# tobiasleibner/dune-hdd

Hardware: AMD Instinct MI355X
Metric: assembled DoFs/sec (global stiffness), SPE10 SWIPDG p=1 (higher is better)
Workload: dtype f64

## Files before the change

dune-hdd_amd/csrc/host/grid.cpp:

```cpp
#include <algorithm>
#include <cmath>
#include <cstring>
#include <fstream>
#include <memory>
#include <numeric>
#include <string>
#include <vector>

#include "hdd.h"
#include "hdd_internal.hh"

namespace hdd {

static const int kSimplexFV[3][2] = {{0, 1}, {0, 2}, {1, 2}};
static const int kCubeFV[4][2] = {{0, 2}, {1, 3}, {0, 1}, {2, 3}};

static inline const int (*face_table(int et))[2] { return et == HDD_SIMPLEX ? kSimplexFV : kCubeFV; }
static inline int nvpe_of(int et) { return et == HDD_SIMPLEX ? 3 : 4; }

static inline double linspace_node(double a, double b, int64_t n, int64_t i)
{
  if (i == n) return b;
  const double step = (b - a) / double(n);
  return double(i) * step + a;
// ... 467 lines not shown
      const double lo = vertex_coords[3 * v[0] + c], hi = vertex_coords[3 * v[1 << c] + c];
      if (!(hi > lo)) return set_error(HDD_ERR_UNSUPPORTED, std::string(fn) + ": element " + std::to_string(e) +
                                                             " is not an axis-aligned box in Dune vertex order");
      for (int k = 0; k < 8; ++k) {
        const double want = ((k >> c) & 1) ? hi : lo, x = vertex_coords[3 * v[k] + c];
        if (std::fabs(x - want) > 1e-12 * std::max(std::fabs(hi - lo), std::fabs(want)))
          return set_error(HDD_ERR_UNSUPPORTED, std::string(fn) + ": element " + std::to_string(e) +
                                                    " is not an axis-aligned box in Dune vertex order");
      }
    }
  }
  auto G = std::make_unique<ExplicitGrid>();
  G->elem_type = HDD_HEX;
  G->dim = 3;
  G->nvpe = 8;
  G->nf = 6;
  G->nb = int(nb);
  return finish_explicit(std::move(G), n_vertices, vertex_coords, n_elements, elem_vert, subdomain, n_subdomains,
                         boundary, out, fn);
}

extern "C" void hdd_grid_destroy(hdd_grid* g) { delete g; }

extern "C" int hdd_grid_get_info(const hdd_grid* g, hdd_grid_info* out)
{
  if (!g || !out) return set_error(HDD_ERR_INVALID, "hdd_grid_get_info: null argument");
  const Grid& G = *g->impl;
  out->elem_type = G.elem_type;
  out->nb = G.nb;
  out->nfaces = G.nf;
  out->nvpe = G.nvpe;
  out->n_elements = G.ne;
  out->n_vertices = G.nv;
  out->n_subdomains = G.n_sub;
  out->dim = G.dim;
  return HDD_OK;
}

extern "C" int hdd_grid_subdomain_range(const hdd_grid* g, int32_t s_begin, int32_t s_end, int64_t* first,
                                        int64_t* last)
{
  if (!g || !first || !last) return set_error(HDD_ERR_INVALID, "hdd_grid_subdomain_range: null argument");
  const Grid& G = *g->impl;
  if (s_begin < 0 || s_end > G.n_sub || s_begin >= s_end)
    return set_error(HDD_ERR_RANGE, "hdd_grid_subdomain_range: 0 <= s_begin < s_end <= num_subdomains violated");
  *first = G.sub_first[s_begin];
// ... 403 lines not shown
```

dune-hdd_amd/csrc/host/hdd_internal.hh:

```
#pragma once
#include <string>

#include "hdd.h"

namespace hdd {
std::string& last_error_slot();
const char*& last_tile_kernel_slot();
int set_error(int code, const std::string& msg);
int ctx_device(const hdd_ctx* ctx);
}

int hdd_fix_rb(int32_t elem_type);
int hdd_assemble_elements_buf(hdd_ctx* ctx, const hdd_mesh* m, const hdd_scalar_fn* kappa, int32_t n_comp,
                              const hdd_tensor_fn* tensor, const hdd_swipdg_params* p, const hdd_csr* pattern,
                              double* const* d_bufs, const int32_t* d_elems, int64_t n_elems, void* stream);
int hdd_scatter_fix(hdd_ctx* ctx, const hdd_csr* pattern, int32_t rb, double* const* d_bufs, int32_t n_comp,
                    const int32_t* d_elems, int64_t n_elems, double* const* d_vals, void* stream);
int hdd_assemble_elements_soa(hdd_ctx* ctx, const hdd_mesh* m, const hdd_scalar_fn* kappa, int32_t n_comp,
                              const hdd_tensor_fn* tensor, const hdd_swipdg_params* p, const hdd_csr* pattern,
                              double* const* d_bufs, int64_t ld, const int32_t* d_elems, int64_t n_elems, void* stream);
int hdd_scatter_fix_q1_soa(hdd_ctx* ctx, const hdd_mesh* m, const hdd_csr* pattern, double* const* d_bufs, int64_t ld,
                           int32_t n_comp, const int32_t* d_elems, int64_t n_elems, double* const* d_vals, void* stream);
int hdd_assemble_reserve(hdd_ctx* ctx, const hdd_mesh* m, const hdd_scalar_fn* kappa, int32_t n_comp,
                         const hdd_tensor_fn* tensor, const hdd_swipdg_params* p, const hdd_csr* pattern,
                         double* const* d_vals, void* stream, int32_t reserve_wg);
int hdd_assemble_elements_inplace(hdd_ctx* ctx, const hdd_mesh* m, const hdd_scalar_fn* kappa, int32_t n_comp,
                                  const hdd_tensor_fn* tensor, const hdd_swipdg_params* p, const hdd_csr* pattern,
                                  double* const* d_vals, const int32_t* d_elems, int64_t n_elems, void* stream);
int hdd_assemble_skip_ghost(hdd_ctx* ctx, const hdd_mesh* m, const hdd_scalar_fn* kappa, int32_t n_comp,
                            const hdd_tensor_fn* tensor, const hdd_swipdg_params* p, const hdd_csr* pattern,
                            double* const* d_vals, void* stream, int32_t reserve_wg = 0);
```

dune-hdd_amd/csrc/kernels/abi_assemble.hip:

```cpp
#include <hip/hip_runtime.h>

#include <algorithm>
#include <cstdint>
#include <string>
#include <vector>

#include "abi_common.hh"
#include "quadrature.hh"

using hdd::set_error;
using namespace hdd::abi;

namespace {
const char* const WHO = "hdd_swipdg_assemble";

struct AssembleMode {
  const int32_t* list = nullptr;
  int64_t n_list = 0;
  int32_t list_kind = hdd::dev::LIST_TILES;
  bool skip_ghost = false;
  int32_t reserve_wg = 0;
  int64_t fix_ld = 0;
};
}

static int assemble_hex(hdd_ctx* ctx, const hdd_mesh* m, const hdd_scalar_fn* kappa, int32_t n_comp,
                        const hdd_tensor_fn* tensor, const hdd_swipdg_params* p, const hdd_csr* pattern,
                        double* const* d_vals, void* stream)
{
  using namespace hdd::dev;
  int deg = 1;
  if (int rc = check_degree(WHO, m, &deg)) return rc;
  if (int rc = check_pattern_rows(WHO, pattern, mesh_nb(HDD_HEX, deg), m)) return rc;
  if (int rc = check_tensor_kind(WHO, tensor)) return rc;
  if (int rc = check_tensor(WHO, tensor)) return rc;
  hipError_t e = hipSetDevice(ctx->device);
  if (e != hipSuccess) return hip_fail(e, "hdd_swipdg_assemble: hipSetDevice");
  for (int c = 0; c < n_comp; ++c) {
    const hdd_scalar_fn& k = kappa[c];
    if (k.kind != HDD_FN_CONST && k.kind != HDD_FN_PER_ELEM && k.kind != HDD_FN_SINUSOID)
      return fail(HDD_ERR_UNSUPPORTED, WHO, "unknown diffusion factor kind");
    if (int rc = check_fn_per_elem(WHO, &k)) return rc;
    if (!d_vals[c]) return fail(HDD_ERR_INVALID, WHO, "null value array");
    const int ko = fn_order(k);
    const int vol_order = p->vol_order >= 0 ? p->vol_order : ko + 2 * (deg - 1);
// ... 72 lines not shown
      return set_error(HDD_ERR_UNSUPPORTED, "hdd_swipdg_assemble_tiles: no tile / element lists for HDD_HEX");
    return assemble_hex(ctx, m, kappa, n_comp, tensor, p, pattern, d_vals, stream);
  }
  int deg = 1;
  if (int rc = check_degree(WHO, m, &deg)) return rc;
  if (int rc = check_pattern_rows(WHO, pattern, mesh_nb(m->elem_type, deg), m)) return rc;
  if (int rc = check_tensor_kind(WHO, tensor)) return rc;
  if (int rc = check_tensor(WHO, tensor)) return rc;
  AssembleArgs a = mesh_args(ctx, m, pattern);
  set_coefficients(a, tensor, p);
  a.n_comp = n_comp;
  a.tile_list = mode.list;
  a.n_tile_list = mode.n_list;
  a.list_elements = mode.list_kind;
  a.skip_ghost = mode.skip_ghost ? 1 : 0;
  a.reserve_wg = mode.list_kind != LIST_TILES ? 0 : mode.reserve_wg;
  a.fix_ld = mode.fix_ld;
  a.fix_rb = hdd_fix_rb(m->elem_type);
  if (int rc = check_vertex_arrays(WHO, m)) return rc;
  if (use_vertex_geometry(ctx, m, false, true)) {
    a.ev = m->elem_vertices;
    a.vxy = m->vertex_coords;
  }
  const int ko = fn_order(kappa[0]);
  for (int c = 0; c < n_comp; ++c) {
    const hdd_scalar_fn& k = kappa[c];
    if (k.kind != HDD_FN_CONST && k.kind != HDD_FN_PER_ELEM && k.kind != HDD_FN_SINUSOID && k.kind != HDD_FN_FLATTOP)
      return fail(HDD_ERR_UNSUPPORTED, WHO, "unknown diffusion factor kind");
    if (int rc = check_fn_per_elem(WHO, &k)) return rc;
    if (fn_order(k) != ko) return fail(HDD_ERR_UNSUPPORTED, WHO, "components of different integration order");
    if (!d_vals[c]) return fail(HDD_ERR_INVALID, WHO, "null value array");
    if (int rc = check_flattop(WHO, &k, m->elem_type, HDD_ERR_INVALID, HDD_ERR_UNSUPPORTED)) return rc;
    a.kappa[c] = KappaArg{k.kind, k.order, k.c, k.b, k.kx, k.ky, k.per_elem, k.table, k.n_table, 0};
    a.vals[c] = d_vals[c];
  }
  const int vol_order = p->vol_order >= 0 ? p->vol_order : ko;
  const int face_order = p->face_order >= 0 ? p->face_order : ko + 2;
  const int nqv = volume_points(m->elem_type, vol_order);
  const int nqf = face_points(face_order);
  bool supported = false;
  hipError_t e = hipSetDevice(ctx->device);
  if (e != hipSuccess) return hip_fail(e, "hdd_swipdg_assemble: hipSetDevice");
  e = launch_assemble(a, nqv, nqf, static_cast<hipStream_t>(stream), &supported);
  if (!supported)
    return set_error(HDD_ERR_UNSUPPORTED, "hdd_swipdg_assemble: no kernel for volume order " + std::to_string(vol_order) +
                                              " / face order " + std::to_string(face_order));
// ... 86 lines not shown
int hdd_assemble_reserve(hdd_ctx* ctx, const hdd_mesh* m, const hdd_scalar_fn* kappa, int32_t n_comp,
                         const hdd_tensor_fn* tensor, const hdd_swipdg_params* p, const hdd_csr* pattern,
                         double* const* d_vals, void* stream, int32_t reserve_wg)
{
  AssembleMode mode;
  mode.reserve_wg = reserve_wg;
  return assemble_impl(ctx, m, kappa, n_comp, tensor, p, pattern, d_vals, mode, stream);
}

int hdd_scatter_fix_q1_soa(hdd_ctx* ctx, const hdd_mesh* m, const hdd_csr* pattern, double* const* d_bufs, int64_t ld,
                           int32_t n_comp, const int32_t* d_elems, int64_t n_elems, double* const* d_vals, void* stream)
{
  if (n_elems == 0) return HDD_OK;
  hdd::dev::AssembleArgs a = mesh_args(ctx, m, pattern);
  a.tile_list = d_elems;
  a.n_tile_list = n_elems;
  for (int32_t c = 0; c < n_comp; ++c) {
    const hipError_t e = hdd::dev::launch_q1_scatter_soa(a, d_bufs[c], ld, d_vals[c], static_cast<hipStream_t>(stream));
    if (e != hipSuccess) return hip_fail(e, "hdd_scatter_fix_q1_soa");
  }
  return HDD_OK;
}

int hdd_assemble_skip_ghost(hdd_ctx* ctx, const hdd_mesh* m, const hdd_scalar_fn* kappa, int32_t n_comp,
                            const hdd_tensor_fn* tensor, const hdd_swipdg_params* p, const hdd_csr* pattern,
                            double* const* d_vals, void* stream, int32_t reserve_wg)
{
  AssembleMode mode;
  mode.skip_ghost = true;
  mode.reserve_wg = reserve_wg;
  return assemble_impl(ctx, m, kappa, n_comp, tensor, p, pattern, d_vals, mode, stream);
}

int hdd_scatter_fix(hdd_ctx* ctx, const hdd_csr* pattern, int32_t rb, double* const* d_bufs, int32_t n_comp,
                    const int32_t* d_elems, int64_t n_elems, double* const* d_vals, void* stream)
{
  if (n_elems == 0) return HDD_OK;
  const unsigned grid = unsigned(std::min<int64_t>(n_elems, int64_t(ctx->n_cu) * 8));
  for (int32_t c = 0; c < n_comp; ++c) {
    hipLaunchKernelGGL(fix_scatter_kernel, dim3(grid), dim3(64), 0, static_cast<hipStream_t>(stream), d_bufs[c], rb,
                       d_elems, n_elems, pattern->elem_ptr, d_vals[c]);
    const hipError_t e = hipGetLastError();
    if (e != hipSuccess) return hip_fail(e, "hdd_scatter_fix");
  }
  return HDD_OK;
}
// ... 1 lines not shown
```

dune-hdd_amd/csrc/kernels/ctx.hh:

```
#pragma once
#include <hip/hip_runtime.h>

#include <cstddef>
#include <cstdint>
#include <string>

#include "hdd.h"
#include "../host/hdd_internal.hh"

#pragma GCC visibility push(hidden)

struct DeviceScratch {
  enum Slack { EXACT, QUARTER };
  enum SyncBeforeFree { NO_SYNC, SYNC_STREAM, SYNC_DEVICE };
  void* p = nullptr;
  size_t bytes = 0;
  const bool pinned_host;

  explicit DeviceScratch(bool pinned_host_ = false) : pinned_host(pinned_host_) {}
  DeviceScratch(const DeviceScratch&) = delete;
  DeviceScratch& operator=(const DeviceScratch&) = delete;
  ~DeviceScratch() { release(); }

  hipError_t reserve(size_t need, Slack slack, SyncBeforeFree sync, hipStream_t s = nullptr)
// ... 32 lines not shown
  int wgcu = 0;
  int q3g_reps = 0;
  double* q3g_tab = nullptr;
  DeviceScratch scan_ws;
  DeviceScratch ops_d;
  DeviceScratch ops_h{true};
  hipEvent_t ops_evt = nullptr;
  int64_t* nnz_h = nullptr;
  int64_t* nnz_hd = nullptr;
  DeviceScratch rhs_ws;
  hipStream_t rhs_stream = nullptr;
  hipEvent_t rhs_evt = nullptr;
  bool rhs_used = false;

  ~hdd_ctx()
  {
    if (q3g_tab) (void)hipFree(q3g_tab);
    if (nnz_h) (void)hipHostFree(nnz_h);
    if (rhs_evt) (void)hipEventDestroy(rhs_evt);
    if (ops_evt) (void)hipEventDestroy(ops_evt);
  }
};

inline bool vx_offsets_fit(int64_t n_local) { return n_local >= 0 && n_local * 48 < (int64_t(1) << 32); }

inline int hip_fail(hipError_t e, const char* where)
{
  return hdd::set_error(HDD_ERR_HIP, std::string(where) + ": " + hipGetErrorString(e));
}

#pragma GCC visibility pop
```

dune-hdd_amd/csrc/kernels/shard.hip:

```cpp
#include <hip/hip_runtime.h>
#include <rccl/rccl.h>

#include <dlfcn.h>

#include <algorithm>
#include <chrono>
#include <condition_variable>
#include <cstdint>
#include <cstring>
#include <map>
#include <mutex>
#include <string>
#include <thread>
#include <vector>

#include "hdd.h"
#include "../host/hdd_internal.hh"

using hdd::set_error;

namespace {

int hip_fail(hipError_t e, const char* where)
{
// ... 591 lines not shown
  if (c->direct && c->direct == static_cast<hipStream_t>(stream)) {
    c->direct = nullptr;
    return HDD_OK;
  }
  hipError_t e = hipSetDevice(c->device);
  if (e == hipSuccess) e = hipStreamWaitEvent(static_cast<hipStream_t>(stream), c->done, 0);
  return e == hipSuccess ? HDD_OK : hip_fail(e, "hdd_comm_wait");
}

struct hdd_shard {
  int device = 0;
  hdd_local* local = nullptr;
  hdd_grid_info gi{};
  hdd_local_info li{};
  int32_t rank = 0, nranks = 1, s_begin = 0, s_end = 0, degree = 1;
  int64_t nnz = 0;
  std::vector<int64_t> gid;
  double* d_coords = nullptr;
  int32_t* d_nbrs = nullptr;
  uint32_t* d_finfo = nullptr;
  int64_t* d_gid = nullptr;
  int32_t* d_ev = nullptr;
  double* d_vxy = nullptr;
  std::vector<int32_t> peers;
  std::vector<int64_t> send_prefix, recv_prefix, recv_col0;
  int32_t* d_send_idx = nullptr;
  double* d_sbuf = nullptr;
  double* d_rbuf = nullptr;
  int32_t max_rows = 0;
  int32_t* d_tiles_in = nullptr;
  int32_t* d_tiles_bd = nullptr;
  int32_t* d_fix = nullptr;
  int64_t n_tiles = 0, n_in = 0, n_bd = 0, n_fix = 0;
  int64_t halo_faces = 0;
  std::vector<int32_t> send_idx, tiles_in, tiles_bd;
  bool host_only = false;
  hipStream_t aux = nullptr;
  hipEvent_t ev_in = nullptr, ev_out = nullptr;
  double* d_fixbuf = nullptr;
  size_t fixbuf_doubles = 0;
  uint32_t stages = 0;
  hipEvent_t ev_pack = nullptr, ev_xdone = nullptr;
  std::vector<int32_t> stage_peers;
  hipEvent_t ev_mark = nullptr;
  bool marked = false;
};
// ... 70 lines not shown
  std::vector<uint32_t> finfo(static_cast<size_t>(nl));
  sh->gid.resize(size_t(nl));
  rc = hdd_local_fill(sh->local, coords.data(), nbrs.data(), finfo.data(), sh->gid.data(), nullptr);
  if (rc) return fail(rc);
  rc = hdd_dg_pattern_count(gi.nfaces, gi.nb, nl, ob, oe, nbrs.data(), &sh->nnz);
  if (rc) return fail(rc);
  std::vector<int32_t> ev;
  std::vector<double> vxy;
  if (gi.dim == 2) {
    int64_t nvl = 0;
    rc = hdd_local_vertices(sh->local, &nvl, nullptr, nullptr);
    if (rc) return fail(rc);
    ev.resize(size_t(gi.nvpe) * nl);
    vxy.resize(size_t(2) * nvl);
    rc = hdd_local_vertices(sh->local, &nvl, ev.data(), vxy.data());
    if (rc) return fail(rc);
  }

  int32_t np = 0;
  rc = hdd_local_halo_plan(sh->local, own.data(), rank, &np, nullptr, nullptr, nullptr, nullptr);
  if (rc) return fail(rc);
  if (np > SH_MAX_PEERS) return fail(set_error(HDD_ERR_UNSUPPORTED, "hdd_shard_create: more than 64 halo peers"));
  sh->peers.resize(size_t(np));
  std::vector<int64_t> sc(static_cast<size_t>(np)), ro(static_cast<size_t>(np)), rcnt(static_cast<size_t>(np));
  rc = hdd_local_halo_plan(sh->local, own.data(), rank, &np, sh->peers.data(), sc.data(), ro.data(), rcnt.data());
  if (rc) return fail(rc);
  sh->send_prefix.assign(size_t(np) + 1, 0);
  sh->recv_prefix.assign(size_t(np) + 1, 0);
  sh->recv_col0 = ro;
  for (int32_t k = 0; k < np; ++k) {
    sh->send_prefix[k + 1] = sh->send_prefix[k] + sc[k];
    sh->recv_prefix[k + 1] = sh->recv_prefix[k] + rcnt[k];
  }
  std::vector<int32_t> send_idx(size_t(sh->send_prefix[np]));
  for (int32_t k = 0; k < np; ++k) {
    if (!sc[k]) continue;
    rc = hdd_local_send_list(sh->local, own.data(), rank, k, send_idx.data() + sh->send_prefix[k]);
    if (rc) return fail(rc);
  }

  const int64_t n_own = oe - ob;
  sh->n_tiles = (n_own + 63) / 64;
  std::vector<int32_t> tin, tbd, fix;
  for (int64_t t = 0; t < sh->n_tiles; ++t) {
    bool ghost = false;
    for (int64_t e = ob + 64 * t; e < std::min(oe, ob + 64 * t + 64); ++e) {
// ... 162 lines not shown
  }
  const hipStream_t s = static_cast<hipStream_t>(stream);

  HaloArgs h{};
  h.ld = sh->li.n_local;
  h.n_peers = int32_t(sh->peers.size());
  auto add = [&](double* p, int rows) {
    h.arr[h.n_arrays] = p;
    h.row_first[h.n_arrays + 1] = h.row_first[h.n_arrays] + rows;
    ++h.n_arrays;
  };
  if (flags & HDD_SHARD_HALO_GEOMETRY) add(sh->d_coords, sh->gi.dim * sh->gi.nvpe);
  if (tensor->kind == HDD_TENSOR_ISO_PER_ELEM || tensor->kind == HDD_TENSOR_SYM_PER_ELEM) {
    if (!tensor->per_elem) return set_error(HDD_ERR_INVALID, "hdd_block_assemble_sharded: tensor per_elem missing");
    add(const_cast<double*>(tensor->per_elem),
        tensor->kind == HDD_TENSOR_ISO_PER_ELEM ? 1 : (sh->gi.dim == 3 ? 6 : 3));
  }
  for (int32_t c = 0; c < n_comp; ++c)
    if (kappa[c].kind == HDD_FN_PER_ELEM) {
      if (!kappa[c].per_elem) return set_error(HDD_ERR_INVALID, "hdd_block_assemble_sharded: kappa per_elem missing");
      add(const_cast<double*>(kappa[c].per_elem), 1);
    }
  const bool exchange = h.n_peers > 0 && !(flags & HDD_SHARD_NO_HALO) && h.n_arrays > 0;
  if (!exchange) return hdd_swipdg_assemble(ctx, &m, kappa, n_comp, tensor, params, pattern, d_vals, stream);
  const bool transfer = !(flags & HDD_SHARD_NO_TRANSFER);
  if (!comm && transfer)
    return set_error(HDD_ERR_INVALID, "hdd_block_assemble_sharded: the shard has halo peers but comm is NULL");
  const int32_t R = h.row_first[h.n_arrays];
  if (R > sh->max_rows) return set_error(HDD_ERR_INVALID, "hdd_block_assemble_sharded: too many halo rows");

  hipError_t e = hipSetDevice(sh->device);
  if (e != hipSuccess) return hip_fail(e, "hdd_block_assemble_sharded: hipSetDevice");
  sh->stages = 0;
  sh->marked = false;
  const bool default_schedule = !(flags & (HDD_SHARD_FIX_INLINE | HDD_SHARD_FIX_SCATTER | HDD_SHARD_FIX_INPLACE));
  const bool split = (flags & HDD_SHARD_SPLIT_TILES) != 0 ||
                     (default_schedule && sh->gi.elem_type == HDD_SIMPLEX && sh->peers.size() >= 2 && sh->n_in > 0);
  const bool q1_serial = sh->gi.elem_type == HDD_CUBE && default_schedule && !(flags & HDD_SHARD_SPLIT_TILES);
  bool overlap = !(flags & HDD_SHARD_NO_OVERLAP) && sh->gi.elem_type != HDD_HEX && !q1_serial &&
                 (split ? sh->n_in > 0 : true);
  hipStream_t ps = s;
#ifdef HDD_ABLATION
  const bool last = (flags & HDD_SHARD_LAUNCH_LAST) != 0;
#else
  const bool last = false;
#endif
  const bool side = overlap && !split;
// ... 257 lines not shown
```

dune-hdd_amd/csrc/kernels/swipdg_kernels.hh:

```
#pragma once
#include <hip/hip_runtime.h>

#include <cstdint>

#include "hdd.h"

namespace hdd {
namespace dev {

struct KappaArg {
  int32_t kind, order;
  double c, b, kx, ky;
  const double* per_elem;
  const double* table;
  int32_t n_table, pad;
};
__host__ __device__ constexpr bool smooth_kind(int k) { return k == HDD_FN_SINUSOID || k == HDD_FN_FLATTOP; }

enum : int32_t {
  LIST_TILES = 0,
  LIST_ELEMENTS = 1,
  LIST_SIDE_BUFFER = 2,
  LIST_IN_PLACE = 3,
  LIST_SIDE_SOA = 4
};

struct AssembleArgs {
  int32_t elem_type, n_comp;
  int64_t n_local, own_begin, own_end;
  const double* coords;
  const int32_t* nbrs;
  const uint32_t* finfo;
  const int64_t* elem_ptr;
  int32_t tkind, n_cu;
  double tc0, tc1, tc2;
  const double* tper;
  double sigma_inner, sigma_boundary, beta;
  int32_t debug_flags, wgcu;
  uint32_t variant;
  int32_t pad_v;
  const int32_t* tile_list;
  int64_t n_tile_list;
  int32_t list_elements;
  int32_t fix_rb;
  int64_t fix_ld;
  int32_t skip_ghost;
  int32_t reserve_wg;
  const int32_t* ev;
  const double* vxy;
  KappaArg kappa[HDD_MAX_COMP];
  double* vals[HDD_MAX_COMP];
};
inline AssembleArgs component_args(const AssembleArgs& a, int c)
{
  AssembleArgs ac = a;
  ac.n_comp = 1;
  ac.kappa[0] = a.kappa[c];
  ac.vals[0] = a.vals[c];
  return ac;
}
template <bool ALL_IN_ONE, class F>
hipError_t per_component(const AssembleArgs& a, F&& launch)
{
  for (int c = 0; c < (ALL_IN_ONE ? 1 : a.n_comp); ++c) {
    launch(ALL_IN_ONE ? a : component_args(a, c));
    const hipError_t e = hipGetLastError();
    if (e != hipSuccess) return e;
  }
  return hipSuccess;
}

struct HexTables {
// ... 108 lines not shown
```

dune-hdd_amd/csrc/kernels/swipdg_launch.hh:

```
#pragma once
#include <algorithm>
#include <string>
#include <type_traits>

#include "hdd_internal.hh"
#include "swipdg_persistent.hh"

namespace hdd {
namespace dev {

template <class P>
static std::string kernel_name(const char* flags)
{
  const std::string f = __PRETTY_FUNCTION__;
  const size_t a = f.find("P = "), b = f.rfind(']');
  std::string p = a == std::string::npos ? "?" : f.substr(a + 4, b - a - 4);
  if (p.rfind("hdd::dev::", 0) == 0) p = p.substr(10);
  return "swipdg_persistent_kernel<" + p + ", " + flags + ">";
}

template <class P>
static hipError_t launch_persistent(const AssembleArgs& a, hipStream_t s)
{
  const int64_t n_own = a.own_end - a.own_begin;
  if (n_own <= 0) return hipSuccess;
  const int64_t tiles = a.tile_list ? a.n_tile_list : (n_own + 63) / 64;
  if (tiles <= 0) return hipSuccess;
  const size_t lds = (P::PAD ? size_t(image_blocks<P>()) * P::RB : size_t(64) * P::RB + 2 + P::RB) * sizeof(double) *
                     (P::TWO ? 2 : 1);
  if (P::TWO && a.n_comp != 2) return hipErrorInvalidValue;
  const int cus = a.n_cu;
  int wgcu = a.wgcu > 0 ? a.wgcu : P::WGCU;
  size_t lds_launch = lds;
#ifdef HDD_ABLATION
  if (a.wgcu >= 16) {
    lds_launch = std::max(lds, size_t((160 * 1024) / (a.wgcu >> 4)) & ~size_t(15));
    wgcu = (a.wgcu & 15) ? (a.wgcu & 15) : P::WGCU;
  }
#endif
  wgcu = std::max(1, std::min<int>(wgcu, int((160 * 1024) / lds_launch)));
  int64_t slots = int64_t(cus) * wgcu;
  const bool reserve = a.reserve_wg > 0 && !HDD_ABL(a, 4194304);
  if (reserve) slots = std::max<int64_t>(8, (slots - a.reserve_wg) & ~int64_t(7));
  const int64_t G = std::min<int64_t>(tiles, slots);
  if (a.list_elements != LIST_TILES) {
    const size_t lds_e = size_t(64) * P::RB * sizeof(double);
    const int64_t ge = std::min<int64_t>((a.n_tile_list + 63) / 64, int64_t(cus) * 4);
    if (a.list_elements >= LIST_SIDE_BUFFER) {
      if (a.list_elements == LIST_SIDE_BUFFER && a.fix_rb != P::RB) return hipErrorInvalidValue;
      if (a.list_elements == LIST_SIDE_SOA && (!P::EMIT || a.fix_ld < a.n_tile_list + 1)) return hipErrorInvalidValue;
      return per_component<P::FUSED>(a, [&](const AssembleArgs& ac) {
        hipLaunchKernelGGL((swipdg_elements_buf_kernel<P>), dim3(unsigned(ge)), dim3(64), 0, s, ac, a.n_tile_list);
      });
    }
    return per_component<P::FUSED>(a, [&](const AssembleArgs& ac) {
      hipLaunchKernelGGL((swipdg_elements_kernel<P>), dim3(unsigned(ge)), dim3(64), lds_e, s, ac, a.n_tile_list);
    });
  }
  static const std::string names[3] = {kernel_name<P>("true, false"), kernel_name<P>("false, true"),
                                       kernel_name<P>("false, false")};
  hdd::last_tile_kernel_slot() = names[a.tile_list ? 0 : (a.skip_ghost ? 1 : 2)].c_str();
  return per_component<P::FUSED>(a, [&](const AssembleArgs& ac) {
    if (a.tile_list)
      hipLaunchKernelGGL((swipdg_persistent_kernel<P, true>), dim3(unsigned(G)), dim3(64), lds_launch, s, ac, tiles);
    else if (a.skip_ghost)
      hipLaunchKernelGGL((swipdg_persistent_kernel<P, false, true>), dim3(unsigned(G)), dim3(64), lds_launch, s, ac, tiles);
    else
// ... 49 lines not shown
```

dune-hdd_amd/csrc/kernels/swipdg_p1.hip:

```cpp
#include "swipdg_policy_p1.hh"
#include "swipdg_policy_generic.hh"
#include "swipdg_launch.hh"

namespace hdd {
namespace dev {

template <int TK, int KK, bool VX> using P1Pwc = P1PwcPolicy<TK, KK, false, VX>;
template <int TK, int KK, bool VX> using P1Smooth3 = GenericPolicy<Simplex, 6, 3, TK, KK, VX>;

static hipError_t dispatch_smooth_p1(const AssembleArgs& a, hipStream_t s)
{
  if (a.variant & HDD_VARIANT_P1_SMOOTH_QUADRATURE) return dispatch_kinds<P1Smooth3>(a, s, true);
  if (a.kappa[0].kind == HDD_FN_FLATTOP) {
    if (!a.ev) return dispatch_kinds<P1Smooth3>(a, s, true);
    return with_tensor_kind(a.tkind, [&](auto tk) {
      return launch_persistent<P1SmoothPolicy<tk.value, true, HDD_FN_FLATTOP>>(a, s);
    });
  }
  return with_tensor_kind(a.tkind, [&](auto tk) {
    return a.ev ? launch_persistent<P1SmoothPolicy<tk.value, true>>(a, s)
                : launch_persistent<P1SmoothPolicy<tk.value>>(a, s);
  });
}

hipError_t launch_p1_pwc(const AssembleArgs& a, hipStream_t s) { return dispatch_kinds<P1Pwc>(a, s, false); }
hipError_t launch_p1_smooth(const AssembleArgs& a, hipStream_t s) { return dispatch_smooth_p1(a, s); }
hipError_t launch_p1_smooth_fused(const AssembleArgs& a, hipStream_t s)
{
  return with_tensor_kind(a.tkind, [&](auto tk) {
    return a.n_comp == 2 ? launch_persistent<P1SmoothFusedPolicy<tk.value, true, true>>(a, s)
                         : launch_persistent<P1SmoothFusedPolicy<tk.value, true>>(a, s);
  });
}

template <int TK, int KK> using P1Pen = P1PwcPolicy<TK, KK, true>;
template <int TK, int KK> using P1PenVX = P1PwcPolicy<TK, KK, true, 1>;
hipError_t launch_p1_penalty(const AssembleArgs& a, hipStream_t s)
{
  return a.ev ? dispatch_pwc<P1PenVX>(a, s) : dispatch_pwc<P1Pen>(a, s);
}

}
}
```

dune-hdd_amd/csrc/kernels/swipdg_policy.hh:

```
#pragma once
#include <hip/hip_runtime.h>

namespace hdd {
namespace dev {

struct PolicyDefaults {
  static constexpr bool FUSED = false;
  struct Shared {};
  static constexpr bool HALF = false;
  static constexpr bool TWO = false;
  static constexpr bool FULLTILE = false;
  static constexpr bool EMIT = false;
};

template <int RB>
struct RotImg {
  double* p;
  int rot;
  __device__ __forceinline__ double& operator[](int i) const
  {
    const unsigned q = unsigned(i + rot);
    return p[q < unsigned(RB) ? q : q - unsigned(RB)];
  }
};

template <class P>
constexpr int image_blocks() { return P::HALF ? 32 : 64; }

}
}
```

dune-hdd_amd/csrc/kernels/swipdg_policy_p1.hh:

```
#pragma once
#include "swipdg_elements.hh"
#include "swipdg_policy.hh"

namespace hdd {
namespace dev {

struct P1Own {
  double X[3], Y[3];
  int32_t nbr[3];
  uint32_t finfo;
  Tensor A;
  double ke;
  int32_t vid[3];
};
struct P1Gat {
  double Ox[3], Oy[3];
  Tensor Ap[3];
  double kn[3];
  int32_t ov[3];
};

template <int TK, int KK, bool VX = false>
__device__ __forceinline__ void p1_load_own(const AssembleArgs& a, int64_t e, P1Own& o)
{
// ... 42 lines not shown
    return;
  }
#pragma unroll
  for (int f = 0; f < 3; ++f) {
    const int64_t n = o.nbr[f] >= 0 ? int64_t(o.nbr[f]) : e;
    const uint32_t inf = (o.finfo >> (4 * f)) & 15u;
    const int tw = int(inf & 7u);
    const int to = 3 - Simplex::fv(tw, 0) - Simplex::fv(tw, 1);
    g.Ox[f] = a.coords[(2 * to) * ne + n];
    g.Oy[f] = a.coords[(2 * to + 1) * ne + n];
    g.Ap[f] = tensor_k<TK>(a, n);
    g.kn[f] = kappa_k<KK>(a, n);
  }
}
template <bool VX>
__device__ __forceinline__ void p1_load_gat2(const AssembleArgs& a, P1Gat& g)
{
  if constexpr (VX) {
#pragma unroll
    for (int f = 0; f < 3; ++f) vertex_xy_o32(a, g.ov[f], g.Ox[f], g.Oy[f]);
  }
}

__device__ __forceinline__ void p1_face_self(double (&S)[3][3], const double (&Ae)[3], int fc, double c, double penT,
                                             double penS)
{
#pragma unroll
  for (int i = 0; i < 3; ++i)
#pragma unroll
    for (int j = i; j < 3; ++j) {
      if (i == fc && j == fc) continue;
      const double v = i == fc ? Ae[i] : (j == fc ? Ae[j] : Ae[i] + Ae[j]);
      S[i][j] = fma(-c, v, S[i][j] + (i == fc || j == fc ? 0.0 : (i == j ? penT : penS)));
    }
}

template <bool PEN = false, bool ALLIN = false>
__device__ __forceinline__ void p1_compute(const AssembleArgs& a, int64_t e, const P1Own& o, const P1Gat& gt,
                                           double* img)
{
  using E = Simplex;
  const double j00 = o.X[1] - o.X[0], j01 = o.X[2] - o.X[0], j10 = o.Y[1] - o.Y[0], j11 = o.Y[2] - o.Y[0];
  const double det = j00 * j11 - j01 * j10;
  const double id = rcp_nr(det);
  const double i00 = j11 * id, i01 = -j01 * id, i10 = -j10 * id, i11 = j00 * id;
  double g[3][2];
  g[1][0] = i00; g[1][1] = i01;
  g[2][0] = i10; g[2][1] = i11;
  g[0][0] = -i00 - i10; g[0][1] = -i01 - i11;
  double Ag[3][2];
#pragma unroll
  for (int k = 0; k < 3; ++k) {
    Ag[k][0] = o.A.a00 * g[k][0] + o.A.a01 * g[k][1];
    Ag[k][1] = o.A.a01 * g[k][0] + o.A.a11 * g[k][1];
  }
  const double adet = fabs(det);
  const double osgn = det > 0.0 ? 1.0 : -1.0;
  const int32_t ei = int32_t(e);
  int nblk = 1, pos_self = 0, pos[3];
#pragma unroll
  for (int f = 0; f < 3; ++f) {
    nblk += ALLIN || o.nbr[f] >= 0;
    pos_self += ((ALLIN || o.nbr[f] >= 0) && o.nbr[f] < ei);
  }
#pragma unroll
  for (int f = 0; f < 3; ++f) {
    int p = (ei < o.nbr[f]) ? 1 : 0;
#pragma unroll
    for (int q = 0; q < 3; ++q) p += ((ALLIN || o.nbr[q] >= 0) && o.nbr[q] < o.nbr[f]);
    pos[f] = p;
  }
  const int rowlen = ALLIN ? 12 : nblk * 3;
  const double ke = o.ke;
  double S[3][3];
  {
    const double fac = PEN ? 0.0 : 0.5 * adet * ke;
#pragma unroll
    for (int i = 0; i < 3; ++i)
#pragma unroll
      for (int j = i; j < 3; ++j) S[i][j] = fac * (Ag[j][0] * g[i][0] + Ag[j][1] * g[i][1]);
  }
  constexpr double CS = PEN ? 0.0 : 1.0;
#pragma unroll
  for (int f = 0; f < 3; ++f) {
    const int32_t n = o.nbr[f];
    if (!ALLIN && n <= HDD_NBR_NEUMANN) continue;
    const int fa = E::fv(f, 0), fb = E::fv(f, 1), fc = 3 - fa - fb;
    const double tx = o.X[fb] - o.X[fa], ty = o.Y[fb] - o.Y[fa];
    const double il = rsq_nr(tx * tx + ty * ty);
    const double len = (tx * tx + ty * ty) * il;
    const double nsc = E::face_sign(f) * osgn * il;
    const double nx = ty * nsc, ny = -tx * nsc;
    double Ae[3];
// ... 30 lines not shown
        double* row = img + i * rowlen + pos[f] * 3;
        if (i == fc) {
          row[jA] = symh * Ae[i];
          row[jB] = symh * Ae[i];
          row[to] = 0.0;
        } else {
          row[jA] = fma(cplh, AnA, fma(symh, Ae[i], -(i == fa ? penT : penS)));
          row[jB] = fma(cplh, AnB, fma(symh, Ae[i], -(i == fb ? penT : penS)));
          row[to] = cplh * AnO;
        }
      }
      p1_face_self(S, Ae, fc, symh, penT, penS);
    } else {
      const double pen = (a.sigma_boundary * ke * dm) * ihp;
      p1_face_self(S, Ae, fc, ke * CS * half, pen * third, pen * sixth);
    }
  }
#pragma unroll
  for (int i = 0; i < 3; ++i)
#pragma unroll
    for (int j = 0; j < 3; ++j) img[i * rowlen + pos_self * 3 + j] = j >= i ? S[i][j] : S[j][i];
}

template <int TK, int KK, bool PEN = false, bool VX = false>
struct P1PwcPolicy : PolicyDefaults {
  static constexpr int NB = 3, NF = 3;
  static constexpr int RB = 36;
  static constexpr int WGCU = VX ? 4 : 8, MINW = 1;
  static constexpr bool PAD = false;
  using Own = P1Own;
  using Gat = P1Gat;
  __device__ static void load_own(const AssembleArgs& a, int64_t e, Own& o) { p1_load_own<TK, KK, VX>(a, e, o); }
  __device__ static void load_gat(const AssembleArgs& a, int64_t e, Own& o, Gat& g) { p1_load_gat<TK, KK, VX>(a, e, o, g); }
  __device__ static void load_gat2(const AssembleArgs& a, Gat& g) { p1_load_gat2<VX>(a, g); }
  __device__ static int n_interior(const Own& o) { return int(o.nbr[0] >= 0) + int(o.nbr[1] >= 0) + int(o.nbr[2] >= 0); }
  __device__ static void compute(const AssembleArgs& a, int64_t e, const Own& o, const Gat& g, double* img)
  {
    p1_compute<PEN>(a, e, o, g, img);
  }
  static constexpr bool FULLTILE = true;
  __device__ static void compute_full(const AssembleArgs& a, int64_t e, const Own& o, const Gat& g, double* img)
  {
    p1_compute<PEN, true>(a, e, o, g, img);
  }
};

template <int TK, bool VX = false, int KK = HDD_FN_SINUSOID>
struct P1SmoothPolicy : PolicyDefaults {
  static constexpr int NB = 3, NF = 3;
  static constexpr int RB = 36;
  static constexpr int WGCU = 8, MINW = 2;
  static constexpr bool PAD = false;
  using Own = P1Own;
  using Gat = P1Gat;
  __device__ static void load_own(const AssembleArgs& a, int64_t e, Own& o) { p1_load_own<TK, HDD_FN_CONST, VX>(a, e, o); }
  __device__ static void load_gat(const AssembleArgs& a, int64_t e, Own& o, Gat& g)
  {
    p1_load_gat<TK, HDD_FN_CONST, VX>(a, e, o, g);
  }
  __device__ static void load_gat2(const AssembleArgs& a, Gat& g) { p1_load_gat2<VX>(a, g); }
  __device__ static int n_interior(const Own& o) { return int(o.nbr[0] >= 0) + int(o.nbr[1] >= 0) + int(o.nbr[2] >= 0); }

  __device__ static void compute(const AssembleArgs& a, int64_t e, const Own& o, const Gat& gt, double* img)
  {
    const KappaArg& K = a.kappa[0];
    auto kap = [&](double x, double y) {
// ... 258 lines not shown
```

Measured before the change: 56.87 billion.

## Recompute Kuhn-triangulation geometry and neighbours in-kernel for structured simplex meshes

At shard creation, the host checks bit-exactly whether the local mesh is a single-partition structured Kuhn triangulation and, if so, stores a compact descriptor. The p1 piecewise-constant assembly kernel then derives vertex coordinates, neighbour indices, face info and neighbour-opposite vertices from the element index, instead of loading them from global memory. Sparse block positions are also computed in closed form for full tiles, replacing comparison loops. The aim is to cut memory traffic and integer work per element. The cost is a one-time host verification pass over all elements and an extra kernel specialization that only handles full tile lists.

```diff
diff --git a/dune-hdd_amd/csrc/host/grid.cpp b/dune-hdd_amd/csrc/host/grid.cpp
--- a/dune-hdd_amd/csrc/host/grid.cpp
+++ b/dune-hdd_amd/csrc/host/grid.cpp
@@ -513,6 +513,12 @@
 
 extern "C" void hdd_grid_destroy(hdd_grid* g) { delete g; }
 
+const hdd_structured_desc* hdd_grid_structured_desc(const hdd_grid* g)
+{
+  const auto* sg = g ? dynamic_cast<const StructuredGrid*>(g->impl.get()) : nullptr;
+  return sg ? &sg->d : nullptr;
+}
+
 extern "C" int hdd_grid_get_info(const hdd_grid* g, hdd_grid_info* out)
 {
   if (!g || !out) return set_error(HDD_ERR_INVALID, "hdd_grid_get_info: null argument");
diff --git a/dune-hdd_amd/csrc/host/hdd_internal.hh b/dune-hdd_amd/csrc/host/hdd_internal.hh
--- a/dune-hdd_amd/csrc/host/hdd_internal.hh
+++ b/dune-hdd_amd/csrc/host/hdd_internal.hh
@@ -8,7 +8,32 @@
 const char*& last_tile_kernel_slot();
 int set_error(int code, const std::string& msg);
 int ctx_device(const hdd_ctx* ctx);
+
+struct KuhnDesc {
+  int32_t nx = 0, ny = 0;
+  double lower[2] = {0.0, 0.0}, step[2] = {0.0, 0.0}, upper[2] = {0.0, 0.0};
+  int32_t bcode = HDD_NBR_DIRICHLET;
+};
+constexpr int32_t KUHN_MIN_NX = 32;
+struct KuhnMeshView {
+  int64_t n_local = 0, own_begin = 0, own_end = 0;
+  int32_t n_peers = 0;
+  const double* coords = nullptr;
+  const int32_t* nbrs = nullptr;
+  const uint32_t* finfo = nullptr;
+  const int32_t* ev = nullptr;
+  const double* vxy = nullptr;
+};
+double kuhn_node(double lower, double step, double upper, int64_t n, int64_t i);
+bool kuhn_detect(const hdd_structured_desc* d, const KuhnMeshView& m, KuhnDesc* out);
 }
+
+inline bool vx_offsets_fit(int64_t n_local) { return n_local >= 0 && n_local * 48 < (int64_t(1) << 32); }
+
+const hdd_structured_desc* hdd_grid_structured_desc(const hdd_grid* g);
+int hdd_assemble_kuhn(hdd_ctx* ctx, const hdd_mesh* m, const hdd_scalar_fn* kappa, int32_t n_comp,
+                      const hdd_tensor_fn* tensor, const hdd_swipdg_params* p, const hdd_csr* pattern,
+                      double* const* d_vals, const hdd::KuhnDesc* kuhn, void* stream);
 
 int hdd_fix_rb(int32_t elem_type);
 int hdd_assemble_elements_buf(hdd_ctx* ctx, const hdd_mesh* m, const hdd_scalar_fn* kappa, int32_t n_comp,
diff --git a/dune-hdd_amd/csrc/host/kuhn.cpp b/dune-hdd_amd/csrc/host/kuhn.cpp
--- /dev/null
+++ b/dune-hdd_amd/csrc/host/kuhn.cpp
@@ -0,0 +1,71 @@
+#include <cstdint>
+#include <cstring>
+
+#include "hdd.h"
+#include "hdd_internal.hh"
+
+namespace hdd {
+
+double kuhn_node(double lower, double step, double upper, int64_t n, int64_t i)
+{
+  if (i == n) return upper;
+  const volatile double p = double(i) * step;
+  return p + lower;
+}
+
+static inline bool same_bits(double a, double b) { return std::memcmp(&a, &b, sizeof(double)) == 0; }
+
+bool kuhn_detect(const hdd_structured_desc* d, const KuhnMeshView& m, KuhnDesc* out)
+{
+  if (!d || !out || d->elem_type != HDD_SIMPLEX || d->px != 1 || d->py != 1) return false;
+  if (d->nx < KUHN_MIN_NX || d->ny < 1) return false;
+  const int64_t nx = d->nx, ny = d->ny, ne = 2 * nx * ny;
+  if (m.n_local != ne || m.own_begin != 0 || m.own_end != ne || m.n_peers != 0) return false;
+  if (!vx_offsets_fit(m.n_local)) return false;
+  if (!m.coords || !m.nbrs || !m.finfo) return false;
+  if (!m.ev != !m.vxy) return false;
+
+  KuhnDesc k;
+  k.nx = d->nx;
+  k.ny = d->ny;
+  for (int c = 0; c < 2; ++c) {
+    k.lower[c] = d->lower[c];
+    k.upper[c] = d->upper[c];
+    k.step[c] = (d->upper[c] - d->lower[c]) / double(c == 0 ? d->nx : d->ny);
+  }
+  k.bcode = d->boundary == HDD_BOUNDARY_ALL_NEUMANN ? HDD_NBR_NEUMANN : HDD_NBR_DIRICHLET;
+  const uint32_t finfo = (2u << 0) | (1u << 4) | (0u << 8);
+
+  auto X = [&](int64_t i) { return kuhn_node(k.lower[0], k.step[0], k.upper[0], nx, i); };
+  auto Y = [&](int64_t j) { return kuhn_node(k.lower[1], k.step[1], k.upper[1], ny, j); };
+  for (int64_t e = 0; e < ne; ++e) {
+    const int64_t sq = e >> 1, i = sq % nx, j = sq / nx;
+    const bool t = (e & 1) != 0;
+    const double vx[3] = {X(i), t ? X(i) : X(i + 1), X(i + 1)};
+    const double vy[3] = {Y(j), t ? Y(j + 1) : Y(j), Y(j + 1)};
+    for (int v = 0; v < 3; ++v) {
+      if (!same_bits(m.coords[(2 * v) * ne + e], vx[v]) || !same_bits(m.coords[(2 * v + 1) * ne + e], vy[v])) return false;
+      if (m.ev) {
+        const int64_t id = m.ev[v * ne + e];
+        if (id < 0 || !same_bits(m.vxy[2 * id], vx[v]) || !same_bits(m.vxy[2 * id + 1], vy[v])) return false;
+      }
+    }
+    const int64_t n0 = t ? (i > 0 ? e - 3 : k.bcode) : (j > 0 ? e - 2 * nx + 1 : k.bcode);
+    const int64_t n1 = e ^ 1;
+    const int64_t n2 = t ? (j < ny - 1 ? e + 2 * nx - 1 : k.bcode) : (i < nx - 1 ? e + 3 : k.bcode);
+    if (m.nbrs[e] != n0 || m.nbrs[ne + e] != n1 || m.nbrs[2 * ne + e] != n2) return false;
+    if (m.finfo[e] != finfo) return false;
+    const int64_t nb[3] = {n0, n1, n2};
+    const double ox[3] = {t ? X(i - 1) : X(i), t ? X(i + 1) : X(i), t ? X(i + 1) : X(i + 2)};
+    const double oy[3] = {t ? Y(j) : Y(j - 1), t ? Y(j) : Y(j + 1), t ? Y(j + 2) : Y(j + 1)};
+    for (int f = 0; f < 3; ++f) {
+      if (nb[f] < 0) continue;
+      if (!same_bits(m.coords[(2 * f) * ne + nb[f]], ox[f]) || !same_bits(m.coords[(2 * f + 1) * ne + nb[f]], oy[f]))
+        return false;
+    }
+  }
+  *out = k;
+  return true;
+}
+
+}
diff --git a/dune-hdd_amd/csrc/kernels/abi_assemble.hip b/dune-hdd_amd/csrc/kernels/abi_assemble.hip
--- a/dune-hdd_amd/csrc/kernels/abi_assemble.hip
+++ b/dune-hdd_amd/csrc/kernels/abi_assemble.hip
@@ -21,6 +21,7 @@
   bool skip_ghost = false;
   int32_t reserve_wg = 0;
   int64_t fix_ld = 0;
+  const hdd::KuhnDesc* kuhn = nullptr;
 };
 }
 
@@ -139,6 +140,10 @@
     a.ev = m->elem_vertices;
     a.vxy = m->vertex_coords;
   }
+  if (mode.kuhn && m->elem_type == HDD_SIMPLEX && m->own_begin == 0 && m->own_end == m->n_local &&
+      m->n_local == int64_t(2) * mode.kuhn->nx * mode.kuhn->ny && mode.kuhn->nx >= hdd::KUHN_MIN_NX &&
+      vx_offsets_fit(m->n_local))
+    a.kuhn = kuhn_args(*mode.kuhn);
   const int ko = fn_order(kappa[0]);
   for (int c = 0; c < n_comp; ++c) {
     const hdd_scalar_fn& k = kappa[c];
@@ -271,6 +276,15 @@
   return HDD_OK;
 }
 
+int hdd_assemble_kuhn(hdd_ctx* ctx, const hdd_mesh* m, const hdd_scalar_fn* kappa, int32_t n_comp,
+                      const hdd_tensor_fn* tensor, const hdd_swipdg_params* p, const hdd_csr* pattern,
+                      double* const* d_vals, const hdd::KuhnDesc* kuhn, void* stream)
+{
+  AssembleMode mode;
+  mode.kuhn = kuhn;
+  return assemble_impl(ctx, m, kappa, n_comp, tensor, p, pattern, d_vals, mode, stream);
+}
+
 int hdd_assemble_skip_ghost(hdd_ctx* ctx, const hdd_mesh* m, const hdd_scalar_fn* kappa, int32_t n_comp,
                             const hdd_tensor_fn* tensor, const hdd_swipdg_params* p, const hdd_csr* pattern,
                             double* const* d_vals, void* stream, int32_t reserve_wg)
diff --git a/dune-hdd_amd/csrc/kernels/ctx.hh b/dune-hdd_amd/csrc/kernels/ctx.hh
--- a/dune-hdd_amd/csrc/kernels/ctx.hh
+++ b/dune-hdd_amd/csrc/kernels/ctx.hh
@@ -78,7 +78,6 @@
   }
 };
 
-inline bool vx_offsets_fit(int64_t n_local) { return n_local >= 0 && n_local * 48 < (int64_t(1) << 32); }
 
 inline int hip_fail(hipError_t e, const char* where)
 {
diff --git a/dune-hdd_amd/csrc/kernels/shard.hip b/dune-hdd_amd/csrc/kernels/shard.hip
--- a/dune-hdd_amd/csrc/kernels/shard.hip
+++ b/dune-hdd_amd/csrc/kernels/shard.hip
@@ -637,6 +637,8 @@
   int64_t* d_gid = nullptr;
   int32_t* d_ev = nullptr;
   double* d_vxy = nullptr;
+  hdd::KuhnDesc kuhn;
+  bool kuhn_on = false;
   std::vector<int32_t> peers;
   std::vector<int64_t> send_prefix, recv_prefix, recv_col0;
   int32_t* d_send_idx = nullptr;
@@ -753,6 +755,19 @@
   if (rc) return fail(rc);
   if (np > SH_MAX_PEERS) return fail(set_error(HDD_ERR_UNSUPPORTED, "hdd_shard_create: more than 64 halo peers"));
   sh->peers.resize(size_t(np));
+  if (gi.dim == 2 && gi.elem_type == HDD_SIMPLEX) {
+    hdd::KuhnMeshView mv;
+    mv.n_local = nl;
+    mv.own_begin = ob;
+    mv.own_end = oe;
+    mv.n_peers = np;
+    mv.coords = coords.data();
+    mv.nbrs = nbrs.data();
+    mv.finfo = finfo.data();
+    mv.ev = ev.data();
+    mv.vxy = vxy.data();
+    sh->kuhn_on = hdd::kuhn_detect(hdd_grid_structured_desc(g), mv, &sh->kuhn);
+  }
   std::vector<int64_t> sc(static_cast<size_t>(np)), ro(static_cast<size_t>(np)), rcnt(static_cast<size_t>(np));
   rc = hdd_local_halo_plan(sh->local, own.data(), rank, &np, sh->peers.data(), sc.data(), ro.data(), rcnt.data());
   if (rc) return fail(rc);
@@ -961,7 +976,10 @@
       add(const_cast<double*>(kappa[c].per_elem), 1);
     }
   const bool exchange = h.n_peers > 0 && !(flags & HDD_SHARD_NO_HALO) && h.n_arrays > 0;
-  if (!exchange) return hdd_swipdg_assemble(ctx, &m, kappa, n_comp, tensor, params, pattern, d_vals, stream);
+  if (!exchange) {
+    const bool kuhn = sh->kuhn_on && !(flags & HDD_SHARD_HALO_GEOMETRY);
+    return hdd_assemble_kuhn(ctx, &m, kappa, n_comp, tensor, params, pattern, d_vals, kuhn ? &sh->kuhn : nullptr, stream);
+  }
   const bool transfer = !(flags & HDD_SHARD_NO_TRANSFER);
   if (!comm && transfer)
     return set_error(HDD_ERR_INVALID, "hdd_block_assemble_sharded: the shard has halo peers but comm is NULL");
diff --git a/dune-hdd_amd/csrc/kernels/swipdg_kernels.hh b/dune-hdd_amd/csrc/kernels/swipdg_kernels.hh
--- a/dune-hdd_amd/csrc/kernels/swipdg_kernels.hh
+++ b/dune-hdd_amd/csrc/kernels/swipdg_kernels.hh
@@ -4,6 +4,7 @@
 #include <cstdint>
 
 #include "hdd.h"
+#include "hdd_internal.hh"
 
 namespace hdd {
 namespace dev {
@@ -24,6 +25,17 @@
   LIST_IN_PLACE = 3,
   LIST_SIDE_SOA = 4
 };
+
+struct KuhnArgs {
+  int32_t on, nx, ny, bcode;
+  uint32_t rnx, pad;
+  double lower[2], step[2], upper[2];
+};
+inline KuhnArgs kuhn_args(const hdd::KuhnDesc& k)
+{
+  return KuhnArgs{1, k.nx, k.ny, k.bcode, uint32_t((uint64_t(1) << 32) / uint64_t(k.nx)), 0u,
+                  {k.lower[0], k.lower[1]}, {k.step[0], k.step[1]}, {k.upper[0], k.upper[1]}};
+}
 
 struct AssembleArgs {
   int32_t elem_type, n_comp;
@@ -48,6 +60,7 @@
   int32_t reserve_wg;
   const int32_t* ev;
   const double* vxy;
+  KuhnArgs kuhn;
   KappaArg kappa[HDD_MAX_COMP];
   double* vals[HDD_MAX_COMP];
 };
diff --git a/dune-hdd_amd/csrc/kernels/swipdg_launch.hh b/dune-hdd_amd/csrc/kernels/swipdg_launch.hh
--- a/dune-hdd_amd/csrc/kernels/swipdg_launch.hh
+++ b/dune-hdd_amd/csrc/kernels/swipdg_launch.hh
@@ -18,6 +18,9 @@
   if (p.rfind("hdd::dev::", 0) == 0) p = p.substr(10);
   return "swipdg_persistent_kernel<" + p + ", " + flags + ">";
 }
+
+template <class P>
+static hipError_t launch_persistent_any(const AssembleArgs& a, hipStream_t s, int64_t tiles, int64_t G, size_t lds_launch);
 
 template <class P>
 static hipError_t launch_persistent(const AssembleArgs& a, hipStream_t s)
@@ -43,6 +46,22 @@
   const bool reserve = a.reserve_wg > 0 && !HDD_ABL(a, 4194304);
   if (reserve) slots = std::max<int64_t>(8, (slots - a.reserve_wg) & ~int64_t(7));
   const int64_t G = std::min<int64_t>(tiles, slots);
+  if constexpr (P::TILES_ONLY) {
+    if (a.tile_list || a.skip_ghost || a.list_elements != LIST_TILES) return hipErrorInvalidValue;
+    static const std::string name = kernel_name<P>("false, false");
+    hdd::last_tile_kernel_slot() = name.c_str();
+    return per_component<P::FUSED>(a, [&](const AssembleArgs& ac) {
+      hipLaunchKernelGGL((swipdg_persistent_kernel<P, false>), dim3(unsigned(G)), dim3(64), lds_launch, s, ac, tiles);
+    });
+  } else {
+    return launch_persistent_any<P>(a, s, tiles, G, lds_launch);
+  }
+}
+
+template <class P>
+static hipError_t launch_persistent_any(const AssembleArgs& a, hipStream_t s, int64_t tiles, int64_t G, size_t lds_launch)
+{
+  const int cus = a.n_cu;
   if (a.list_elements != LIST_TILES) {
     const size_t lds_e = size_t(64) * P::RB * sizeof(double);
     const int64_t ge = std::min<int64_t>((a.n_tile_list + 63) / 64, int64_t(cus) * 4);
diff --git a/dune-hdd_amd/csrc/kernels/swipdg_p1.hip b/dune-hdd_amd/csrc/kernels/swipdg_p1.hip
--- a/dune-hdd_amd/csrc/kernels/swipdg_p1.hip
+++ b/dune-hdd_amd/csrc/kernels/swipdg_p1.hip
@@ -23,7 +23,13 @@
   });
 }
 
-hipError_t launch_p1_pwc(const AssembleArgs& a, hipStream_t s) { return dispatch_kinds<P1Pwc>(a, s, false); }
+template <int TK, int KK> using P1PwcKuhn = P1PwcPolicy<TK, KK, false, true, true>;
+hipError_t launch_p1_pwc(const AssembleArgs& a, hipStream_t s)
+{
+  if (a.kuhn.on && a.ev && !a.tile_list && !a.skip_ghost && a.list_elements == LIST_TILES)
+    return dispatch_pwc<P1PwcKuhn>(a, s);
+  return dispatch_kinds<P1Pwc>(a, s, false);
+}
 hipError_t launch_p1_smooth(const AssembleArgs& a, hipStream_t s) { return dispatch_smooth_p1(a, s); }
 hipError_t launch_p1_smooth_fused(const AssembleArgs& a, hipStream_t s)
 {
diff --git a/dune-hdd_amd/csrc/kernels/swipdg_policy.hh b/dune-hdd_amd/csrc/kernels/swipdg_policy.hh
--- a/dune-hdd_amd/csrc/kernels/swipdg_policy.hh
+++ b/dune-hdd_amd/csrc/kernels/swipdg_policy.hh
@@ -11,6 +11,7 @@
   static constexpr bool TWO = false;
   static constexpr bool FULLTILE = false;
   static constexpr bool EMIT = false;
+  static constexpr bool TILES_ONLY = false;
 };
 
 template <int RB>
diff --git a/dune-hdd_amd/csrc/kernels/swipdg_policy_p1.hh b/dune-hdd_amd/csrc/kernels/swipdg_policy_p1.hh
--- a/dune-hdd_amd/csrc/kernels/swipdg_policy_p1.hh
+++ b/dune-hdd_amd/csrc/kernels/swipdg_policy_p1.hh
@@ -88,6 +88,66 @@
   }
 }
 
+template <bool LAST = true>
+__device__ __forceinline__ double kuhn_node(int32_t i, int32_t n, double lower, double step, double upper)
+{
+  const double p = double(i) * step;
+  const double x = p + lower;
+  if constexpr (!LAST) return x;
+  return i == n ? upper : x;
+}
+template <int TK, int KK>
+__device__ __forceinline__ void p1_load_own_kuhn(const AssembleArgs& a, int64_t e, P1Own& o)
+{
+  const KuhnArgs& k = a.kuhn;
+  const uint32_t eu = uint32_t(e), nx = uint32_t(k.nx);
+  const uint32_t e0 = __builtin_amdgcn_readfirstlane(eu);
+  const uint32_t sq0 = e0 >> 1;
+  uint32_t j0 = __umulhi(sq0, k.rnx), i0 = sq0 - j0 * nx;
+  if (i0 >= nx) {
+    i0 -= nx;
+    ++j0;
+  }
+  const uint32_t iu = i0 + ((eu - e0) >> 1);
+  const bool wrap = iu >= nx;
+  const int32_t i = int32_t(wrap ? iu - nx : iu), j = int32_t(j0) + (wrap ? 1 : 0);
+  const bool t = (eu & 1u) != 0u;
+  o.vid[0] = i; o.vid[1] = j; o.vid[2] = t ? 1 : 0;
+  const int32_t ei = int32_t(eu), w = 2 * k.nx;
+  const bool in0 = t ? i > 0 : j > 0, in2 = t ? j < k.ny - 1 : i < k.nx - 1;
+  o.nbr[0] = in0 ? ei + (t ? -3 : 1 - w) : k.bcode;
+  o.nbr[1] = ei ^ 1;
+  o.nbr[2] = in2 ? ei + (t ? w - 1 : 3) : k.bcode;
+  o.finfo = (2u << 0) | (1u << 4) | (0u << 8);
+  const double x0 = kuhn_node<false>(i, k.nx, k.lower[0], k.step[0], k.upper[0]);
+  const double x1 = kuhn_node(i + 1, k.nx, k.lower[0], k.step[0], k.upper[0]);
+  const double y0 = kuhn_node<false>(j, k.ny, k.lower[1], k.step[1], k.upper[1]);
+  const double y1 = kuhn_node(j + 1, k.ny, k.lower[1], k.step[1], k.upper[1]);
+  o.X[0] = x0; o.Y[0] = y0;
+  o.X[1] = t ? x0 : x1; o.Y[1] = t ? y1 : y0;
+  o.X[2] = x1; o.Y[2] = y1;
+  o.A = tensor_o32<TK>(a, 8u * eu);
+  o.ke = kappa_o32<KK>(a, 8u * eu);
+}
+template <int TK, int KK>
+__device__ __forceinline__ void p1_load_gat_kuhn(const AssembleArgs& a, int64_t e, const P1Own& o, P1Gat& g)
+{
+  const KuhnArgs& k = a.kuhn;
+#pragma unroll
+  for (int f = 0; f < 3; ++f) {
+    const uint32_t n = o.nbr[f] >= 0 ? uint32_t(o.nbr[f]) : uint32_t(e);
+    g.Ap[f] = tensor_o32<TK>(a, 8u * n);
+    g.kn[f] = kappa_o32<KK>(a, 8u * n);
+  }
+  const int32_t i = o.vid[0], j = o.vid[1];
+  const bool t = o.vid[2] != 0;
+  const double xo = kuhn_node(t ? i - 1 : i + 2, k.nx, k.lower[0], k.step[0], k.upper[0]);
+  const double yo = kuhn_node(t ? j + 2 : j - 1, k.ny, k.lower[1], k.step[1], k.upper[1]);
+  g.Ox[0] = t ? xo : o.X[0];     g.Oy[0] = t ? o.Y[0] : yo;
+  g.Ox[1] = t ? o.X[2] : o.X[0]; g.Oy[1] = t ? o.Y[0] : o.Y[2];
+  g.Ox[2] = t ? o.X[2] : xo;     g.Oy[2] = t ? yo : o.Y[2];
+}
+
 __device__ __forceinline__ void p1_face_self(double (&S)[3][3], const double (&Ae)[3], int fc, double c, double penT,
                                              double penS)
 {
@@ -101,7 +161,7 @@
     }
 }
 
-template <bool PEN = false, bool ALLIN = false>
+template <bool PEN = false, bool ALLIN = false, bool KPOS = false>
 __device__ __forceinline__ void p1_compute(const AssembleArgs& a, int64_t e, const P1Own& o, const P1Gat& gt,
                                            double* img)
 {
@@ -124,17 +184,23 @@
   const double osgn = det > 0.0 ? 1.0 : -1.0;
   const int32_t ei = int32_t(e);
   int nblk = 1, pos_self = 0, pos[3];
-#pragma unroll
-  for (int f = 0; f < 3; ++f) {
-    nblk += ALLIN || o.nbr[f] >= 0;
-    pos_self += ((ALLIN || o.nbr[f] >= 0) && o.nbr[f] < ei);
-  }
-#pragma unroll
-  for (int f = 0; f < 3; ++f) {
-    int p = (ei < o.nbr[f]) ? 1 : 0;
-#pragma unroll
-    for (int q = 0; q < 3; ++q) p += ((ALLIN || o.nbr[q] >= 0) && o.nbr[q] < o.nbr[f]);
-    pos[f] = p;
+  if constexpr (KPOS && ALLIN) {
+    const int t = ei & 1;
+    pos_self = 1 + t;
+    pos[0] = 0; pos[1] = 2 - t; pos[2] = 3;
+  } else {
+#pragma unroll
+    for (int f = 0; f < 3; ++f) {
+      nblk += ALLIN || o.nbr[f] >= 0;
+      pos_self += ((ALLIN || o.nbr[f] >= 0) && o.nbr[f] < ei);
+    }
+#pragma unroll
+    for (int f = 0; f < 3; ++f) {
+      int p = (ei < o.nbr[f]) ? 1 : 0;
+#pragma unroll
+      for (int q = 0; q < 3; ++q) p += ((ALLIN || o.nbr[q] >= 0) && o.nbr[q] < o.nbr[f]);
+      pos[f] = p;
+    }
   }
   const int rowlen = ALLIN ? 12 : nblk * 3;
   const double ke = o.ke;
@@ -211,17 +277,30 @@
     for (int j = 0; j < 3; ++j) img[i * rowlen + pos_self * 3 + j] = j >= i ? S[i][j] : S[j][i];
 }
 
-template <int TK, int KK, bool PEN = false, bool VX = false>
+template <int TK, int KK, bool PEN = false, bool VX = false, bool KUHN = false>
 struct P1PwcPolicy : PolicyDefaults {
+  static_assert(!KUHN || (VX && !PEN), "implicit Kuhn geometry: the vertex-indexed stiffness policy");
+  static constexpr bool TILES_ONLY = KUHN;
   static constexpr int NB = 3, NF = 3;
   static constexpr int RB = 36;
   static constexpr int WGCU = VX ? 4 : 8, MINW = 1;
   static constexpr bool PAD = false;
   using Own = P1Own;
   using Gat = P1Gat;
-  __device__ static void load_own(const AssembleArgs& a, int64_t e, Own& o) { p1_load_own<TK, KK, VX>(a, e, o); }
-  __device__ static void load_gat(const AssembleArgs& a, int64_t e, Own& o, Gat& g) { p1_load_gat<TK, KK, VX>(a, e, o, g); }
-  __device__ static void load_gat2(const AssembleArgs& a, Gat& g) { p1_load_gat2<VX>(a, g); }
+  __device__ static void load_own(const AssembleArgs& a, int64_t e, Own& o)
+  {
+    if constexpr (KUHN) p1_load_own_kuhn<TK, KK>(a, e, o);
+    else p1_load_own<TK, KK, VX>(a, e, o);
+  }
+  __device__ static void load_gat(const AssembleArgs& a, int64_t e, Own& o, Gat& g)
+  {
+    if constexpr (KUHN) p1_load_gat_kuhn<TK, KK>(a, e, o, g);
+    else p1_load_gat<TK, KK, VX>(a, e, o, g);
+  }
+  __device__ static void load_gat2(const AssembleArgs& a, Gat& g)
+  {
+    if constexpr (!KUHN) p1_load_gat2<VX>(a, g);
+  }
   __device__ static int n_interior(const Own& o) { return int(o.nbr[0] >= 0) + int(o.nbr[1] >= 0) + int(o.nbr[2] >= 0); }
   __device__ static void compute(const AssembleArgs& a, int64_t e, const Own& o, const Gat& g, double* img)
   {
@@ -230,7 +309,7 @@
   static constexpr bool FULLTILE = true;
   __device__ static void compute_full(const AssembleArgs& a, int64_t e, const Own& o, const Gat& g, double* img)
   {
-    p1_compute<PEN, true>(a, e, o, g, img);
+    p1_compute<PEN, true, KUHN>(a, e, o, g, img);
   }
 };
 
```

Measured after the change: 54.19 billion. 0.953x the previous value.
